# MaurizioFD/RecSys2019_DeepLearning_Evaluation

Measured on AMD Instinct MI355X. Metric: BPR-MF SGD samples/sec (k=128, batch 1000) + ItemKNN cosine build sec on ML-20M-shaped URM, higher is better.
Workload: dtype f32; 1 GPU; BPR-MF epoch (139 mini-batches x 1000 on-device samples), k=128, sgd, on synthetic ml20m URM 138493x26744 nnz=20001422; replicas (one independent model per GPU); batch_size=1000, n_factors=128, parallelism=replicas x1

## Files before the change

include/mi355rec.h:

```cpp
#ifndef MI355REC_H
#define MI355REC_H

#include <stdint.h>

#ifdef __cplusplus
extern "C" {
#endif

#define MI355REC_OK              0
#define MI355REC_E_INVALID      -1
#define MI355REC_E_HIP          -2
#define MI355REC_E_NO_DEVICE    -3
#define MI355REC_E_UNSUPPORTED  -4
#define MI355REC_E_NUMERIC      -5

const char *mi355rec_last_error(void);

int mi355rec_device_malloc(void **out, uint64_t bytes);
int mi355rec_device_free(void *p);
int mi355rec_device_memcpy(void *dst, const void *src, uint64_t bytes, int to_device);
int mi355rec_device_synchronize(void);
int mi355rec_device_trim(uint64_t *freed_bytes);
int mi355rec_device_count(int *count);
int mi355rec_set_device(int device);
// ... 108 lines not shown
    uint64_t random_seed;
    int32_t precision;
    int32_t reserved;
} mi355rec_mf_config;

typedef struct mi355rec_mf *mi355rec_mf_t;

int mi355rec_mf_create(mi355rec_mf_t *out, const mi355rec_mf_config *cfg, int32_t n_users, int32_t n_items,
                       const int32_t *indptr, const int32_t *indices, const float *data,
                       const void *U0, const void *V0);
int mi355rec_mf_run_epochs(mi355rec_mf_t h, int32_t n_epochs);
int mi355rec_mf_run_samples(mi355rec_mf_t h, const int32_t *u, const int32_t *i, const int32_t *j,
                            const float *rating, int64_t n);
int mi355rec_mf_shard_begin_epoch(mi355rec_mf_t h, int32_t rank, int32_t world, void **d_send, void **d_recv,
                                  uint64_t *bytes_per_rank, int32_t *n_batches);
int mi355rec_mf_shard_batch(mi355rec_mf_t h, int32_t batch);
int mi355rec_mf_shard_merge(mi355rec_mf_t h, int32_t batch);
int mi355rec_mf_shard_end_epoch(mi355rec_mf_t h);
int mi355rec_mf_get_factors(mi355rec_mf_t h, float *U, float *V, float *bu, float *bi, float *mu);
int mi355rec_mf_get_factors_f64(mi355rec_mf_t h, double *U, double *V, double *bu, double *bi, double *mu);
int mi355rec_mf_get_last_samples(mi355rec_mf_t h, int32_t *u, int32_t *i, int32_t *j, float *rating, int64_t cap, int64_t *n);
int mi355rec_mf_set_profiling(mi355rec_mf_t h, int32_t max_timed_launches);
int mi355rec_mf_get_phase_ticks(mi355rec_mf_t h, uint64_t *out, int64_t cap, int64_t *n);
int mi355rec_mf_get_stats(mi355rec_mf_t h, mi355rec_stats *stats);
void mi355rec_mf_destroy(mi355rec_mf_t h);

typedef struct mi355rec_mf_group *mi355rec_mf_group_t;
int mi355rec_mf_group_create(mi355rec_mf_group_t *out, const mi355rec_mf_t *members, int32_t n_members);
int mi355rec_mf_group_run_epochs(mi355rec_mf_group_t g, int32_t n_epochs);
int mi355rec_mf_group_set_profiling(mi355rec_mf_group_t g, int32_t max_timed_launches);
int mi355rec_mf_group_get_stats(mi355rec_mf_group_t g, mi355rec_stats *stats);
void mi355rec_mf_group_destroy(mi355rec_mf_group_t g);


typedef struct {
    int32_t symmetric;
    int32_t sgd_mode;
    double  learning_rate, li_reg, lj_reg;
    double  gamma, beta_1, beta_2;
    uint64_t random_seed;
    int32_t precision;
    int32_t train_with_sparse_weights;
    int32_t topK;
    int32_t reserved;
} mi355rec_slim_config;

// ... 201 lines not shown
```

recsys2019_deeplearning_evaluation_amd/_native.py:

```python
import ctypes as C
import os

import numpy as np

_HERE = os.path.dirname(os.path.abspath(__file__))
LIB_PATH = os.environ.get("MI355REC_LIB") or os.path.join(_HERE, "libmi355rec.so")

E_INVALID, E_HIP, E_NO_DEVICE, E_UNSUPPORTED, E_NUMERIC = -1, -2, -3, -4, -5

SIMILARITY_CODES = {"cosine": 0, "adjusted": 1, "asymmetric": 2, "pearson": 3, "jaccard": 4, "tanimoto": 4,
                    "dice": 5, "tversky": 6, "euclidean": 7}
EUCLIDEAN_MODE_CODES = {"lin": 0, "log": 1, "exp": 2}
FEATURE_WEIGHTING_CODES = {"none": 0, "BM25": 1, "TF-IDF": 2}
SGD_MODE_CODES = {"sgd": 0, "adagrad": 1, "rmsprop": 2, "adam": 3}
ALGORITHM_CODES = {"MF_BPR": 0, "FUNK_SVD": 1, "ASY_SVD": 2}
PRECISION_CODES = {"fp32": 0, "fp64": 1}


class NativeLibraryError(RuntimeError):
    """libmi355rec.so is missing, or the HIP runtime / device failed."""


class Stats(C.Structure):
    _fields_ = [("call_ms", C.c_double), ("kernel_ms", C.c_double), ("n_launches", C.c_int64), ("n_timed", C.c_int64),
# ... 63 lines not shown
    "mi355rec_sim_compute_dense_device": (C.c_int, [_vp, _i32, _i32, _vp, _i64]),
    "mi355rec_sim_compute_csr": (C.c_int, [_vp, C.c_int32, C.c_int32, _vp, _vp, _vp, _vp]),
    "mi355rec_sim_column_costs": (C.c_int, [_vp, _vp]),
    "mi355rec_sim_schedule_info": (C.c_int, [_vp, _vp, _vp, _vp]),
    "mi355rec_sim_accumulator_info": (C.c_int, [_vp, C.POINTER(_i32), C.POINTER(_f64)]),
    "mi355rec_sim_selection_info": (C.c_int, [_vp, C.POINTER(_i64), C.POINTER(_i64), C.POINTER(_i64)]),
    "mi355rec_lds_atomic_rate": (C.c_int, [C.POINTER(_f64)]),
    "mi355rec_sim_sync": (C.c_int, [_vp]),
    "mi355rec_sim_get_stats": (C.c_int, [_vp, C.POINTER(Stats)]),
    "mi355rec_sim_destroy": (None, [_vp]),
    "mi355rec_csr_stack_device": (C.c_int, [_i32, C.POINTER(CsrBlock), _i32, _vp, _vp, _vp]),
    "mi355rec_mf_create": (C.c_int, [C.POINTER(_vp), C.POINTER(MFConfig), _i32, _i32, _vp, _vp, _vp, _vp, _vp]),
    "mi355rec_mf_run_epochs": (C.c_int, [_vp, _i32]),
    "mi355rec_mf_run_samples": (C.c_int, [_vp, _vp, _vp, _vp, _vp, _i64]),
    "mi355rec_mf_shard_begin_epoch": (C.c_int, [_vp, _i32, _i32, C.POINTER(_vp), C.POINTER(_vp), C.POINTER(C.c_uint64), C.POINTER(_i32)]),
    "mi355rec_mf_shard_batch": (C.c_int, [_vp, _i32]),
    "mi355rec_mf_shard_merge": (C.c_int, [_vp, _i32]),
    "mi355rec_mf_shard_end_epoch": (C.c_int, [_vp]),
    "mi355rec_mf_get_factors": (C.c_int, [_vp, _vp, _vp, _vp, _vp, _vp]),
    "mi355rec_mf_get_factors_f64": (C.c_int, [_vp, _vp, _vp, _vp, _vp, _vp]),
    "mi355rec_mf_get_last_samples": (C.c_int, [_vp, _vp, _vp, _vp, _vp, _i64, C.POINTER(_i64)]),
    "mi355rec_mf_set_profiling": (C.c_int, [_vp, _i32]),
    "mi355rec_mf_get_phase_ticks": (C.c_int, [_vp, _vp, _i64, C.POINTER(_i64)]),
    "mi355rec_mf_get_stats": (C.c_int, [_vp, C.POINTER(Stats)]),
    "mi355rec_mf_destroy": (None, [_vp]),
    "mi355rec_mf_group_create": (C.c_int, [C.POINTER(_vp), C.POINTER(_vp), _i32]),
    "mi355rec_mf_group_run_epochs": (C.c_int, [_vp, _i32]),
    "mi355rec_mf_group_set_profiling": (C.c_int, [_vp, _i32]),
    "mi355rec_mf_group_get_stats": (C.c_int, [_vp, C.POINTER(Stats)]),
    "mi355rec_mf_group_destroy": (None, [_vp]),
    "mi355rec_slim_create": (C.c_int, [C.POINTER(_vp), C.POINTER(SlimConfig), _i32, _i32, _vp, _vp]),
    "mi355rec_slim_run_epochs": (C.c_int, [_vp, _i32]),
    "mi355rec_slim_run_samples": (C.c_int, [_vp, _vp, _vp, _vp, _i64]),
    "mi355rec_slim_get_last_samples": (C.c_int, [_vp, _vp, _vp, _vp, _i64, C.POINTER(_i64)]),
    "mi355rec_slim_get_S_topk": (C.c_int, [_vp, _i32, _vp, _vp]),
    "mi355rec_slim_get_W_csr": (C.c_int, [_vp, _i32, _vp, _vp, _vp, _vp, _vp, C.POINTER(C.c_int64)]),
    "mi355rec_slim_get_S_sparse": (C.c_int, [_vp, _vp, _vp]),
    "mi355rec_slim_get_S_dense": (C.c_int, [_vp, _vp]),
    "mi355rec_slim_get_stats": (C.c_int, [_vp, C.POINTER(Stats)]),
    "mi355rec_slim_schedule_info": (C.c_int, [_vp, C.POINTER(_i32), C.POINTER(_i32)]),
    "mi355rec_slim_destroy": (None, [_vp]),
    "mi355rec_ials_create": (C.c_int, [C.POINTER(_vp), _i32, _i32, _i32, _f64, _vp, _vp, _vp, _vp, _vp]),
    "mi355rec_ials_run_epochs": (C.c_int, [_vp, _i32]),
    "mi355rec_ials_user_half": (C.c_int, [_vp, _i32, _i32]),
    "mi355rec_ials_item_half": (C.c_int, [_vp, _i32, _i32]),
    "mi355rec_ials_device_factors": (C.c_int, [_vp, C.POINTER(_vp), C.POINTER(_vp)]),
# ... 391 lines not shown
```

recsys2019_deeplearning_evaluation_amd/csrc/mf.hip:

```cpp
#include "common.h"
#include "sampling.cuh"
#include "wave.cuh"

#include <rocprim/rocprim.hpp>

#include <memory>

#include "mf_core.cuh"
#include "mf_schedule.cuh"
#include "mf_batch.cuh"
#include "mf_asy.cuh"


using namespace mi355rec;

struct mi355rec_mf : Handle {
    mi355rec_mf_config cfg{};
    int n_users = 0, n_items = 0, k = 0;
    int n_u_rows = 0;
    bool f64 = false;
    size_t nnz = 0;
    DeviceBuffer<int> indptr, indices, su, si, sj;
    DeviceBuffer<float> data, sr, stage;
    DeviceBuffer<unsigned char> U[2], V[2], bu[2], bi[2], c1U, c2U, c1V, c2V, c1_bu, c2_bu, c1_bi, c2_bi;
    DeviceBuffer<unsigned char> mu_state, mu_acc, asy_mu, asy_c_mu;
    DeviceBuffer<unsigned char> par;
    DeviceBuffer<double> loss_slots;
    DeviceBuffer<MfState> state;
    DeviceBuffer<unsigned long long> keys, keys_sorted;
    DeviceBuffer<int> slots, slots_sorted, head, head_scan, task_at, batch_count;
    DeviceBuffer<unsigned char> spar, cub_tmp;
    DeviceBuffer<TaskHeader> tasks;
    DeviceBuffer<unsigned> touched;
    DeviceBuffer<int> sorted_slot, qtask, used;
    bool fast_schedule = false;
    DeviceBuffer<unsigned long long> ticks;
    DeviceBuffer<int4> recs, slot_recs;
    size_t cub_tmp_bytes = 0;
    size_t stream_capacity = 0;
    long long batch_capacity = 0;
    long long batches_done = 0;
    long long last_call_samples = 0;
    int max_timed = 0;
    DeviceBuffer<unsigned char> shard_send, shard_recv;
    int shard_rank = -1, shard_world = 0, shard_slots_per_rank = 0;
    long long shard_batches = 0;
    std::vector<hipGraphExec_t> epoch_graphs;
    size_t general_capacity = 0;
    bool graph_failed = false;
    std::vector<double> host_loss;

    void drop_graphs() {
        for (hipGraphExec_t g : epoch_graphs) (void)hipGraphExecDestroy(g);
        epoch_graphs.clear();
    }
    ~mi355rec_mf() { shutdown([&] { drop_graphs(); }); }
};

namespace {
// ... 157 lines not shown
}

FastSchedParams fast_sched_params(mi355rec_mf *h, long long n_samples) {
    FastSchedParams f;
    memset(&f, 0, sizeof(f));
    f.n_samples = n_samples;
    f.per = per_sample(h);
    f.n_users = h->n_users;
    f.n_entries = h->n_users + h->n_items;
    f.batch_size = h->cfg.batch_size;
    f.tasks_per_batch = f.per * h->cfg.batch_size;
    f.np = std::max(SCHED_THREADS, pow2_at_least(f.tasks_per_batch));
    f.slot_bits = bits_for((unsigned long long)f.np);
    f.entry_bits = std::min(32 - f.slot_bits, bits_for((unsigned long long)f.n_entries) + 1);
    f.mid_bytes = (int)sched_mid_bytes(f.np);
    f.words = FAST_MAX_BATCHES / 32;
    f.group = samples_in_flight(h);
    f.su = h->su.ptr; f.si = h->si.ptr; f.sj = h->sj.ptr; f.sr = h->sr.ptr;
    f.touched = h->touched.ptr; f.par = h->par.ptr;
    f.sorted_slot = h->sorted_slot.ptr; f.qtask = h->qtask.ptr; f.used = h->used.ptr;
    f.tasks = h->tasks.ptr; f.recs = h->recs.ptr; f.slot_recs = h->slot_recs.ptr;
    f.fuse = h->cfg.algorithm == MI355REC_MF_BPR && h->shard_rank < 0 && !getenv("MI355REC_MF_NO_FUSE");
    f.fill_all = 1;
    return f;
}

void enqueue_fast_schedule(mi355rec_mf *h, long long n_samples, long long n_batches, const FastSchedParams *given = nullptr,
                           hipStream_t on = nullptr) {
    hipStream_t s = on ? on : h->stream;
    const FastSchedParams f = given ? *given : fast_sched_params(h, n_samples);
    const size_t lds = sched_lds_bytes(f.np);
    static bool attr_set[64] = {};
    set_sched_sort_attribute(reinterpret_cast<const void *>(mf_sched_sort_kernel), attr_set);
    hipLaunchKernelGGL(mf_sched_sort_kernel, dim3((unsigned)n_batches), dim3(SCHED_THREADS), lds, s, f);
    hipLaunchKernelGGL(mf_sched_emit_kernel, dim3(div_up(f.batch_size, 256), (unsigned)n_batches), dim3(256), 0, s, f);
    hipLaunchKernelGGL(mf_sched_finish_kernel, dim3(div_up(f.n_entries, 256)), dim3(256), 0, s, f);
}

void enqueue_schedule(mi355rec_mf *h, long long n_samples, long long n_batches) {
    if (h->fast_schedule && fast_schedule_fits(h, n_batches)) {
        enqueue_fast_schedule(h, n_samples, n_batches);
        return;
    }
    hipStream_t s = h->stream;
    const int per = per_sample(h);
    const long long n = n_samples * per;
    SchedParams sp{};
// ... 17 lines not shown
    MI_REQUIRE(end_bit <= 64, "sample stream too long for the schedule keys");
    MI_HIP(hipMemsetAsync(h->batch_count.ptr, 0, sizeof(int) * (size_t)n_batches, s));
    MI_HIP(hipMemsetAsync(h->tasks.ptr, 0, sizeof(TaskHeader) * (size_t)n_batches * sp.tasks_per_batch, s));
    hipLaunchKernelGGL(mf_keys_kernel, dim3(div_up(n_samples, 256)), dim3(256), 0, s, sp);
    size_t bytes = h->cub_tmp_bytes;
    MI_HIP(rocprim::radix_sort_pairs(h->cub_tmp.ptr, bytes, h->keys.ptr, h->keys_sorted.ptr, h->slots.ptr,
                                              h->slots_sorted.ptr, (int)n, 0, end_bit, s));
    MI_HIP(hipMemsetAsync(sp.slot_flag, 0, sizeof(int) * (size_t)n, s));
    hipLaunchKernelGGL(mf_heads_kernel, dim3(div_up(n, 256)), dim3(256), 0, s, sp);
    bytes = h->cub_tmp_bytes;
    MI_HIP(rocprim::inclusive_scan(h->cub_tmp.ptr, bytes, h->head.ptr, h->head_scan.ptr, (size_t)n, rocprim::plus<int>(), s));
    bytes = h->cub_tmp_bytes;
    MI_HIP(rocprim::exclusive_scan(h->cub_tmp.ptr, bytes, sp.slot_flag, reinterpret_cast<int *>(h->keys.ptr) + n, 0, (size_t)n, rocprim::plus<int>(), s));
    hipLaunchKernelGGL(mf_tasks_kernel, dim3(div_up(n, 256)), dim3(256), 0, s, sp);
    hipLaunchKernelGGL(mf_recs_kernel, dim3(div_up(n, 256)), dim3(256), 0, s, sp);
}

long long schedule_span(const mi355rec_mf *h, long long n_batches) {
    if (h->shard_rank < 0 && n_batches > FAST_MAX_BATCHES && fast_schedule_fits(h, 1) && !getenv("MI355REC_MF_WHOLE_STREAM_SCHEDULE"))
        return FAST_MAX_BATCHES;
    return n_batches;
}

template <class T>
void enqueue_stream(mi355rec_mf *h, const MfParams<T> &p, long long n_samples, long long n_batches, bool timed, long long first = 0,
                    long long last = -1) {
    const bool bpr = h->cfg.algorithm == MI355REC_MF_BPR;
    const long long span = schedule_span(h, n_batches), B = h->cfg.batch_size;
    if (last < 0) last = n_batches;
    for (long long b = first; b < last; ++b) {
        const long long part = b / span * span, local = b - part, part_batches = std::min(span, n_batches - part);
        if (local == 0) {
            if (span == n_batches) {
                enqueue_schedule(h, n_samples, n_batches);
            } else {
                FastSchedParams f = fast_sched_params(h, std::min(n_samples - part * B, part_batches * B));
                f.su += part * B; f.si += part * B; f.sj += part * B; f.sr += part * B;
                enqueue_fast_schedule(h, f.n_samples, part_batches, &f);
            }
        }
        if (bpr) launch_batch<MI355REC_MF_BPR, T>(h, p, (int)local, timed);
        else launch_batch<MI355REC_MF_FUNK_SVD, T>(h, p, (int)local, timed);
        if (local + 1 == part_batches) hipLaunchKernelGGL(mf_stream_end_kernel<T>, dim3(1), dim3(64), 0, h->stream, p, part_batches);
    }
}

constexpr int ASY_CHUNK = 1 << 16;

template <class T>
void enqueue_asy_steps(mi355rec_mf *h, const MfParams<T> &p, long long n_steps, bool timed) {
    for (long long first = 0; first < n_steps; first += ASY_CHUNK) {
        const int count = (int)std::min<long long>(ASY_CHUNK, n_steps - first);
        hipEvent_t e0 = nullptr, e1 = nullptr;
        if (timed) h->dispatch_timers.next(e0, e1, h->max_timed);
        auto go = [&](auto kernel) {
            if (e0) hipExtLaunchKernelGGL(kernel, dim3(1), dim3(1024), 0, h->stream, e0, e1, 0, p, first, count);
            else hipLaunchKernelGGL(kernel, dim3(1), dim3(1024), 0, h->stream, p, first, count);
        };
        if (h->k <= 64) go(mf_asy_kernel<T, 1>);
        else if (h->k <= 128) go(mf_asy_kernel<T, 2>);
        else go(mf_asy_kernel<T, 4>);
    }
}

template <class T>
void enqueue_epoch(mi355rec_mf *h, const MfParams<T> &p, bool timed, long long first = 0, long long last = -1) {
    if (first == 0) launch_sampler(h, p);
    if (h->cfg.algorithm == MI355REC_MF_ASY_SVD) {
        enqueue_asy_steps(h, p, p.samples_per_epoch, timed);
        return;
    }
    enqueue_stream(h, p, p.samples_per_epoch, batches_per_epoch(h), timed, first, last);
}

constexpr long long GRAPH_SEGMENT = 4096, MAX_GRAPH_BATCHES = 64 * GRAPH_SEGMENT;
template <class T>
void ensure_epoch_graph(mi355rec_mf *h, const MfParams<T> &p) {
    if (!h->epoch_graphs.empty() || h->graph_failed) return;
    const long long nb = h->cfg.algorithm == MI355REC_MF_ASY_SVD ? 1 : batches_per_epoch(h);
    for (long long first = 0; first < nb; first += GRAPH_SEGMENT) {
        hipGraph_t g = nullptr;
        hipGraphExec_t exec = nullptr;
        hipError_t e = hipStreamBeginCapture(h->stream, hipStreamCaptureModeThreadLocal);
        if (e == hipSuccess) {
            try {
                enqueue_epoch(h, p, false, first, std::min(nb, first + GRAPH_SEGMENT));
            } catch (...) {
                (void)hipStreamEndCapture(h->stream, &g);
                if (g) (void)hipGraphDestroy(g);
                (void)hipGetLastError();
                h->drop_graphs();
                h->graph_failed = true;
                return;
            }
            e = hipStreamEndCapture(h->stream, &g);
// ... 221 lines not shown
        MI_REQUIRE(cfg->sgd_mode >= MI355REC_SGD && cfg->sgd_mode <= MI355REC_ADAM, "Value for 'sgd_mode' not recognized (%d)",
                   cfg->sgd_mode);
        MI_REQUIRE(cfg->n_factors >= 1, "n_factors must be >= 1");
        if (cfg->n_factors > 512) fail(MI355REC_E_UNSUPPORTED, "n_factors = %d exceeds 512", cfg->n_factors);
        MI_REQUIRE(cfg->batch_size >= 1, "batch_size must be >= 1");
        MI_REQUIRE(cfg->precision == MI355REC_F32 || cfg->precision == MI355REC_F64, "precision must be MI355REC_F32 or MI355REC_F64");
        ensure_device();
        std::unique_ptr<mi355rec_mf> h(new mi355rec_mf());
        h->cfg = *cfg;
        h->n_users = n_users;
        h->n_items = n_items;
        h->k = cfg->n_factors;
        h->n_u_rows = asy ? n_items : n_users;
        h->f64 = cfg->precision == MI355REC_F64;
        h->nnz = (size_t)indptr[n_users];
        MI_REQUIRE(h->nnz > 0, "URM has no interactions");
        h->open(1);
        hipStream_t s = h->stream;
        h->indptr.upload(indptr, (size_t)n_users + 1, s);
        h->indices.upload(indices, h->nnz, s);
        h->data.upload(data, h->nnz, s);
        if (h->f64) create_typed<double>(h.get(), U0, V0); else create_typed<float>(h.get(), U0, V0);
        h->par.alloc_zero((size_t)n_users + n_items, s);
        if (getenv("MI355REC_MF_TICKS")) h->ticks.alloc_zero((size_t)per_sample(h.get()) * cfg->batch_size * 8, s);
        h->loss_slots.alloc_zero((size_t)per_sample(h.get()) * cfg->batch_size * 4, s);
        h->state.alloc_zero(1, s);
        {
            MfState init{};
            init.beta_1_power = cfg->beta_1;
            init.beta_2_power = cfg->beta_2;
            MI_HIP(hipMemcpyAsync(h->state.ptr, &init, sizeof(MfState), hipMemcpyHostToDevice, s));
        }
        MI_HIP(hipStreamSynchronize(s));
        *out = h.release();
    });
}

extern "C" int mi355rec_mf_run_epochs(mi355rec_mf_t h, int32_t n_epochs) {
    return guarded([&] {
        MI_REQUIRE(h, "NULL handle");
        MI_REQUIRE(n_epochs >= 0, "n_epochs must be >= 0");
        ensure_device();
        ReleaseScope scope(h->stream);
        if (h->f64) run_epochs_typed<double>(h, n_epochs); else run_epochs_typed<float>(h, n_epochs);
    });
}

// ... 503 lines not shown

extern "C" int mi355rec_mf_set_profiling(mi355rec_mf_t h, int32_t max_timed_launches) {
    return guarded([&] {
        MI_REQUIRE(h, "NULL handle");
        MI_REQUIRE(max_timed_launches >= 0 && max_timed_launches <= 65536, "max_timed_launches out of range");
        ensure_device();
        h->max_timed = max_timed_launches;
        h->dispatch_timers.reserve(max_timed_launches);
    });
}

extern "C" int mi355rec_mf_get_phase_ticks(mi355rec_mf_t h, uint64_t *out, int64_t cap, int64_t *n) {
    return guarded([&] {
        MI_REQUIRE(h && n, "NULL argument");
        ensure_device();
        *n = (int64_t)h->ticks.count;
        if (out && cap > 0) {
            MI_HIP(hipStreamSynchronize(h->stream));
            MI_HIP(hipMemcpy(out, h->ticks.ptr, sizeof(uint64_t) * std::min<size_t>((size_t)cap, h->ticks.count), hipMemcpyDeviceToHost));
        }
    });
}

extern "C" int mi355rec_mf_get_stats(mi355rec_mf_t h, mi355rec_stats *stats) { return handle_get_stats(h, stats); }

extern "C" void mi355rec_mf_destroy(mi355rec_mf_t h) { handle_destroy(h); }
```

recsys2019_deeplearning_evaluation_amd/csrc/mf_core.cuh:

```cuda
#pragma once

namespace mi355rec {
namespace {


struct MfState {
    long long batch_base;
    long long epoch;
    double beta_1_power, beta_2_power;
    double asy_loss;
};

struct TaskHeader {
    int entry;
    int meta;
    int start;
    int pad;
    int4 rec0;
};
constexpr int LEN_MASK = 0x0fffffff;
typedef int int8v __attribute__((ext_vector_type(8)));
constexpr int ROLE_U = 0, ROLE_I = 1;

template <class T> struct MuState { T mu, c1, c2, pad; };
// ... 73 lines not shown

template <class T> __device__ __forceinline__ T grad_term(T scale, T x, T reg, T w) {
#pragma clang fp contract(off)
    const T a = scale * x;
    const T b = reg * w;
    return a - b;
}
__device__ __forceinline__ float fused_add(float a, float b, float c) { return __builtin_fmaf(a, b, c); }
__device__ __forceinline__ double fused_add(double a, double b, double c) { return __builtin_fma(a, b, c); }
template <class T> __device__ __forceinline__ T diff_of(T a, T b) {
#pragma clang fp contract(off)
    return a - b;
}
template <class T> __device__ __forceinline__ T mean_of(T sum, T inv_batch) {
#pragma clang fp contract(off)
    return sum * inv_batch;
}
template <class T> __device__ __forceinline__ T moved(T w, T lr, T step) {
#pragma clang fp contract(off)
    const T a = lr * step;
    return w + a;
}

template <int ALGO, class T>
__device__ __forceinline__ void mf_sample_body(const MfParams<T> &p) {
    const long long t = blockIdx.x * (long long)blockDim.x + threadIdx.x;
    const long long epoch = p.state->epoch;
    if (t < p.samples_per_epoch) {
        const unsigned long long sid = (unsigned long long)(epoch * p.samples_per_epoch + t);
        unsigned d = 0;
        int u, start = 0, n_seen = 0;
        do {
            u = bounded(draw32(p.seed, sid, d++), p.n_users);
            start = p.indptr[u];
            n_seen = p.indptr[u + 1] - start;
        } while (n_seen == 0 || n_seen == p.n_items);
        const int *row = p.indices + start;
        p.su[t] = u;
        if (ALGO == MI355REC_MF_BPR) {
            p.si[t] = row[bounded(draw32(p.seed, sid, d++), n_seen)];
            int j;
            do { j = bounded(draw32(p.seed, sid, d++), p.n_items); } while (!profile_lacks(row, n_seen, j));
            p.sj[t] = j;
        } else {
            bool positive = true;
            if (p.sample_negatives) positive = (float)draw32(p.seed, sid, d++) * 2.3283064365386963e-10f <= p.quota;
            if (positive) {
                const int at = bounded(draw32(p.seed, sid, d++), n_seen);
                p.si[t] = row[at];
                p.sr[t] = p.data[start + at];
            } else {
                int i;
                do { i = bounded(draw32(p.seed, sid, d++), p.n_items); } while (!profile_lacks(row, n_seen, i));
                p.si[t] = i;
                p.sr[t] = 0.f;
            }
        }
    }
}
template <int ALGO, class T>
__global__ __launch_bounds__(256) void mf_sample_kernel(const MfParams<T> p) { mf_sample_body<ALGO, T>(p); }
__global__ void mf_epoch_advance_kernel(MfState *state) {
    if (threadIdx.x == 0 && blockIdx.x == 0) state->epoch += 1;
}

}
}
```

recsys2019_deeplearning_evaluation_amd/csrc/mf_schedule.cuh:

```cuda
#pragma once

namespace mi355rec {
namespace {

struct SchedParams {
    long long n_samples;
    int per;
    int n_users, batch_size, batch_bits, tasks_per_batch;
    const int *su, *si, *sj;
    const float *sr;
    unsigned long long *keys;
    int *slots;
    const unsigned long long *keys_sorted;
    const int *slots_sorted;
    int *head;
    const int *head_scan;
    int *task_at;
    unsigned char *spar;
    unsigned char *par;
    int *batch_count;
    int *slot_flag;
    const int *slot_rank;
    TaskHeader *tasks;
    int4 *recs;
// ... 62 lines not shown
    if (q >= n) return;
    const int slot = s.slots_sorted[q];
    const int sample = slot / s.per, role = slot - sample * s.per;
    const long long base = (long long)sample * s.per;
    int4 rec;
    rec.x = s.su[sample];
    rec.y = s.si[sample];
    rec.z = s.per == 3 ? s.sj[sample] : __float_as_int(s.sr[sample]);
    rec.w = role | (s.spar[base] << 2) | (s.spar[base + 1] << 3) | (s.per == 3 ? s.spar[base + 2] << 4 : 0);
    s.recs[q] = rec;
    if (s.head[q]) {
        s.tasks[s.task_at[q]].rec0 = rec;
        const int entry = (int)(s.keys_sorted[q] >> s.batch_bits);
        long long end = q + 1;
        while (end < n && !s.head[end]) ++end;
        if (end == n || (int)(s.keys_sorted[end] >> s.batch_bits) != entry) s.par[entry] = s.spar[slot] ^ 1;
    }
}

constexpr int META_WIDE = 1 << 30;
constexpr int SCHED_THREADS = 1024;
constexpr int SLOT_ABSORBED = 0x3fffffff;
constexpr int FAST_MAX_BATCHES = 256, FAST_MAX_SLOTS = 8192;

struct FastSchedParams {
    long long n_samples;
    int per, n_users, n_entries, batch_size, tasks_per_batch, slot_bits, np, words, group;
    int fill_all;
    int mid_bytes;
    int entry_bits;
    int fuse;
    const int *su, *si, *sj;
    const float *sr;
    unsigned *touched;
    unsigned char *par;
    int *sorted_slot;
    int *qtask;
    int *used;
    TaskHeader *tasks;
    int4 *recs;
    int4 *slot_recs;
};

template <int IPT> struct SchedSort {
    using type = rocprim::block_radix_sort<unsigned, SCHED_THREADS, IPT>;
    static __device__ __forceinline__ void run(unsigned *K, void *storage, int begin_bit, int end_bit) {
        unsigned keys[IPT];
#pragma unroll
        for (int i = 0; i < IPT; ++i) keys[i] = K[threadIdx.x * IPT + i];
        type().sort(keys, *reinterpret_cast<typename type::storage_type *>(storage), (unsigned)begin_bit, (unsigned)end_bit);
        __syncthreads();
#pragma unroll
        for (int i = 0; i < IPT; ++i) K[threadIdx.x * IPT + i] = keys[i];
    }
};
constexpr size_t sched_sort_storage_bytes(int np) {
    return np <= SCHED_THREADS ? sizeof(SchedSort<1>::type::storage_type)
           : (np <= 2 * SCHED_THREADS ? sizeof(SchedSort<2>::type::storage_type)
              : (np <= 4 * SCHED_THREADS ? sizeof(SchedSort<4>::type::storage_type) : sizeof(SchedSort<8>::type::storage_type)));
}

__device__ __forceinline__ void mf_sched_sort_body(const FastSchedParams &s, const int b) {
    extern __shared__ __attribute__((aligned(16))) unsigned sched_lds[];
    unsigned *K = sched_lds;
    int *hpos = reinterpret_cast<int *>(sched_lds + s.np);
    int *tpos = hpos + s.np + 1;
    typedef rocprim::block_scan<int, SCHED_THREADS> Scan;
    __shared__ typename Scan::storage_type scan_tmp;
    const int tid = threadIdx.x, np = s.np, sb = s.slot_bits;
    const long long first = (long long)b * s.batch_size;
    const int n_in = (int)min((long long)s.batch_size, s.n_samples - first);
    const int m = n_in * s.per;
    for (int q = tid; q < np; q += SCHED_THREADS) {
        unsigned key = 0xFFFFFFFFu;
        if (q < m) {
            const int smp = q / s.per, role = q - smp * s.per;
            const long long t = first + smp;
            const int entry = role == 0 ? s.su[t] : s.n_users + (role == 1 ? s.si[t] : s.sj[t]);
            key = ((unsigned)entry << sb) | (unsigned)q;
        }
        K[q] = key;
    }
    __syncthreads();
    switch (np / SCHED_THREADS) {
        case 1: SchedSort<1>::run(K, hpos, sb, sb + s.entry_bits); break;
        case 2: SchedSort<2>::run(K, hpos, sb, sb + s.entry_bits); break;
        case 4: SchedSort<4>::run(K, hpos, sb, sb + s.entry_bits); break;
        default: SchedSort<8>::run(K, hpos, sb, sb + s.entry_bits); break;
    }
    __syncthreads();
    const int C = np / SCHED_THREADS;
    int cnt = 0;
    for (int c = 0; c < C; ++c) {
        const int q = tid * C + c;
        cnt += q < m && (q == 0 || (K[q] >> sb) != (K[q - 1] >> sb));
    }
    int off = 0, total = 0;
    Scan().exclusive_scan(cnt, off, 0, total, scan_tmp);
    for (int c = 0; c < C; ++c) {
        const int q = tid * C + c;
        if (q < m && (q == 0 || (K[q] >> sb) != (K[q - 1] >> sb))) hpos[off++] = q;
    }
    if (tid == 0) hpos[total] = m;
    __syncthreads();
    unsigned char *single = reinterpret_cast<unsigned char *>(sched_lds) + sizeof(unsigned) * (size_t)np + s.mid_bytes;
    const unsigned qmask = (1u << sb) - 1u;
    if (s.fuse) {
        for (int q = tid; q < np; q += SCHED_THREADS) single[q] = 0;
        __syncthreads();
        for (int t = tid; t < total; t += SCHED_THREADS)
            if (hpos[t + 1] - hpos[t] == 1) single[K[hpos[t]] & qmask] = 1;
        __syncthreads();
    }
    auto absorbed = [&](int t) -> bool {
        if (!s.fuse || hpos[t + 1] - hpos[t] != 1) return false;
        const int inc = (int)(K[hpos[t]] & qmask), smp = inc / s.per;
        return inc != smp * s.per && single[smp * s.per];
    };
    auto lone_user = [&](int q) -> bool {
        if (q >= m) return false;
        const unsigned e = K[q] >> sb;
        return e < (unsigned)s.n_users && (q == 0 || (K[q - 1] >> sb) != e) && (q + 1 == m || (K[q + 1] >> sb) != e);
    };
    auto paired = [&](int q) -> bool {
        if (!s.fuse || s.group < 2) return false;
        const int q0 = q - q % s.group;
        for (int e = 0; e < s.group; ++e)
            if (!lone_user(q0 + e)) return false;
        return true;
    };
    const int CT = (total + SCHED_THREADS - 1) / SCHED_THREADS;
    const int t_lo = min(tid * CT, total), t_hi = min(t_lo + CT, total);
    int wcnt = 0, acnt = 0;
    const int wide_min = 2 * s.group;
    for (int t = t_lo; t < t_hi; ++t) {
        const int start = hpos[t], len = hpos[t + 1] - start;
        wcnt += len > wide_min;
        acnt += absorbed(t) || (len == 1 && start % s.group != 0 && paired(start));
    }
    int woff = 0, n_wide = 0, aoff = 0, n_abs = 0;
    Scan().exclusive_scan(wcnt, woff, 0, n_wide, scan_tmp);
    __syncthreads();
    Scan().exclusive_scan(acnt, aoff, 0, n_abs, scan_tmp);
    TaskHeader *out = s.tasks + (size_t)b * s.tasks_per_batch;
    for (int t = t_lo; t < t_hi; ++t) {
        const int start = hpos[t], len = hpos[t + 1] - start;
        const bool wide = len > wide_min;
        const int entry = (int)(K[start] >> sb);
        atomicOr(&s.touched[(size_t)entry * s.words + (b >> 5)], 1u << (b & 31));
        const bool pair = len == 1 && paired(start);
        if (absorbed(t) || (pair && start % s.group != 0)) {
            ++aoff;
            tpos[t] = SLOT_ABSORBED;
            continue;
        }
        const int slot = wide ? 4 * woff : 4 * n_wide + (t - woff - aoff);
        woff += wide;
        tpos[t] = slot | (wide ? META_WIDE : 0);
        for (int part = 0; part < (wide ? 4 : 1); ++part) {
            *reinterpret_cast<int4 *>(out + slot + part) =
                make_int4(entry, (pair ? s.group : len) | (wide ? META_WIDE | (part << 28) : 0), b * s.tasks_per_batch + start, pair ? 1 : 0);
            out[slot + part].rec0 = make_int4(0, 0, 0, 0);
        }
    }
    const int used = 4 * n_wide + (total - n_wide - n_abs);
    if (tid == 0) s.used[b] = used;
    const int fill_end = s.fill_all ? s.tasks_per_batch : min(s.tasks_per_batch, (used + 3) & ~3);
    for (int slot = used + tid; slot < fill_end; slot += SCHED_THREADS)
        *reinterpret_cast<int4 *>(out + slot) = make_int4(0, 0, 0, 0);
    __syncthreads();
    for (int q = tid; q < m; q += SCHED_THREADS) {
        int lo = 0, hi = total;
        while (hi - lo > 1) {
            const int mid = (lo + hi) >> 1;
            if (hpos[mid] <= q) lo = mid; else hi = mid;
        }
        const int inc = (int)(K[q] & qmask);
        int also = 0;
        if (s.fuse && hpos[lo + 1] - hpos[lo] == 1) {
            const int smp = inc / s.per;
            if (inc == smp * s.per) also = (single[inc + 1] ? 1 : 0) | (s.per == 3 && single[inc + 2] ? 2 : 0);
        }
        s.sorted_slot[(size_t)b * s.tasks_per_batch + inc] = q | (also << 16);
        s.qtask[(size_t)b * s.tasks_per_batch + q] = tpos[lo];
    }
}
__global__ __launch_bounds__(SCHED_THREADS) void mf_sched_sort_kernel(const FastSchedParams s) { mf_sched_sort_body(s, blockIdx.x); }

__device__ __forceinline__ int version_parity(const FastSchedParams &s, int entry, int b) {
    const unsigned *w = s.touched + (size_t)entry * s.words;
    int cnt = 0;
    for (int k = 0; k < (b >> 5); ++k) cnt += __popc(w[k]);
    cnt += __popc(w[b >> 5] & ((1u << (b & 31)) - 1u));
    return (s.par[entry] + cnt) & 1;
}

__device__ __forceinline__ void mf_sched_emit_body(const FastSchedParams &s) {
    const int b = blockIdx.y, smp = blockIdx.x * 256 + threadIdx.x;
    const long long first = (long long)b * s.batch_size;
    const int n_in = (int)min((long long)s.batch_size, s.n_samples - first);
    if (smp >= n_in) return;
    const size_t base = (size_t)b * s.tasks_per_batch;
    const long long t = first + smp;
    const int u = s.su[t], i = s.si[t], j = s.per == 3 ? s.sj[t] : 0;
    const int third = s.per == 3 ? j : __float_as_int(s.sr[t]);
    int where[3];
#pragma unroll
    for (int role = 0; role < 3; ++role) where[role] = role < s.per ? s.sorted_slot[base + (size_t)smp * s.per + role] : 0;
    const int pu = version_parity(s, u, b), pi = version_parity(s, s.n_users + i, b);
    const int pj = s.per == 3 ? version_parity(s, s.n_users + j, b) : 0;
    const int par_bits = (pu << 2) | (pi << 3) | (pj << 4);
#pragma unroll
    for (int role = 0; role < 3; ++role) {
        if (role >= s.per) break;
        const int q = where[role] & 0xffff, also = where[role] >> 16;
        const size_t at = base + q;
        const int4 rec = make_int4(u, i, third, role | par_bits | (also << 5));
        s.recs[at] = rec;
        const int tp = s.qtask[at];
        if (tp == SLOT_ABSORBED) {
            const int q0 = q - q % s.group;
            if (s.fuse && q0 != q) {
                const int tp0 = s.qtask[base + q0];
                if (tp0 != SLOT_ABSORBED && !(tp0 & META_WIDE)) {
                    const TaskHeader *lead = s.tasks + base + tp0;
                    if (lead->pad == 1 && lead->start == (int)(base + q0)) s.slot_recs[(base + tp0) * 3 + (q - q0 - 1)] = rec;
                }
            }
            continue;
        }
        TaskHeader *hd = s.tasks + base + (tp & (META_WIDE - 1));
        const int off = (int)(at - (size_t)hd->start);
        const int own = role == 0 ? pu : (role == 1 ? pi : pj);
        int part = -1;
        if (tp & META_WIDE) {
            if (off % s.group == 0 && off / s.group < 4) part = off / s.group;
        } else if (off == 0) {
            part = 0;
        }
        if (part >= 0) {
            hd[part].rec0 = rec;
            hd[part].meta |= own << 31;
        }
    }
}

__global__ __launch_bounds__(256) void mf_sched_emit_kernel(const FastSchedParams s) { mf_sched_emit_body(s); }

__device__ __forceinline__ void mf_sched_finish_body(const FastSchedParams &s) {
    const int x = blockIdx.x * 256 + threadIdx.x;
    if (x >= s.n_entries) return;
    unsigned *w = s.touched + (size_t)x * s.words;
    int cnt = 0;
    for (int k = 0; k < s.words; ++k) {
        const unsigned v = w[k];
        if (v) { cnt += __popc(v); w[k] = 0; }
    }
    if (cnt & 1) s.par[x] ^= 1;
}
__global__ __launch_bounds__(256) void mf_sched_finish_kernel(const FastSchedParams s) { mf_sched_finish_body(s); }

template <class T>
__device__ __forceinline__ void ring_to_stream_start(const MfParams<T> &p, const long long n_batches, const int slot) {
    if (n_batches <= 0) return;
    const int src = (int)((n_batches - 1) % 3);
    if (src != 2) {
        if (slot == 0) p.mu_state[2] = p.mu_state[src];
        p.mu_acc[2 * MU_SLOTS + slot] = p.mu_acc[src * MU_SLOTS + slot];
    }
    p.mu_acc[slot] = (T)0;
}

template <class T>
// ... 17 lines not shown
```

Measured before the change: 225.9 million samples/s.

## Fuse BPR sample drawing into schedule sort kernel and streamline emit lookups

When the whole epoch fits the fast schedule, the separate sampler kernel launch is skipped and samples are drawn inside the per-batch schedule sort kernel, which writes the sort keys directly. The finish kernel advances the epoch counter instead. The emit kernel now loads touched bitmaps as uint4 with an unrolled popcount, and reads the task offset and pair flag packed into qtask rather than dereferencing task headers. Optional schedule timestamp probes are added behind an env var. The risks are heavier work per sort block, since drawing is serialised into 1024-thread blocks per batch, and the hardcoded 8-word bitmap stride and packed qtask bit fields.

```diff
diff --git a/include/mi355rec.h b/include/mi355rec.h
--- a/include/mi355rec.h
+++ b/include/mi355rec.h
@@ -154,6 +154,7 @@
 int mi355rec_mf_get_last_samples(mi355rec_mf_t h, int32_t *u, int32_t *i, int32_t *j, float *rating, int64_t cap, int64_t *n);
 int mi355rec_mf_set_profiling(mi355rec_mf_t h, int32_t max_timed_launches);
 int mi355rec_mf_get_phase_ticks(mi355rec_mf_t h, uint64_t *out, int64_t cap, int64_t *n);
+int mi355rec_mf_get_schedule_ticks(mi355rec_mf_t h, uint64_t *out, int64_t cap, int64_t *n);
 int mi355rec_mf_get_stats(mi355rec_mf_t h, mi355rec_stats *stats);
 void mi355rec_mf_destroy(mi355rec_mf_t h);
 
diff --git a/recsys2019_deeplearning_evaluation_amd/_native.py b/recsys2019_deeplearning_evaluation_amd/_native.py
--- a/recsys2019_deeplearning_evaluation_amd/_native.py
+++ b/recsys2019_deeplearning_evaluation_amd/_native.py
@@ -109,6 +109,7 @@
     "mi355rec_mf_get_last_samples": (C.c_int, [_vp, _vp, _vp, _vp, _vp, _i64, C.POINTER(_i64)]),
     "mi355rec_mf_set_profiling": (C.c_int, [_vp, _i32]),
     "mi355rec_mf_get_phase_ticks": (C.c_int, [_vp, _vp, _i64, C.POINTER(_i64)]),
+    "mi355rec_mf_get_schedule_ticks": (C.c_int, [_vp, _vp, _i64, C.POINTER(_i64)]),
     "mi355rec_mf_get_stats": (C.c_int, [_vp, C.POINTER(Stats)]),
     "mi355rec_mf_destroy": (None, [_vp]),
     "mi355rec_mf_group_create": (C.c_int, [C.POINTER(_vp), C.POINTER(_vp), _i32]),
diff --git a/recsys2019_deeplearning_evaluation_amd/csrc/mf.hip b/recsys2019_deeplearning_evaluation_amd/csrc/mf.hip
--- a/recsys2019_deeplearning_evaluation_amd/csrc/mf.hip
+++ b/recsys2019_deeplearning_evaluation_amd/csrc/mf.hip
@@ -34,7 +34,7 @@
     DeviceBuffer<unsigned> touched;
     DeviceBuffer<int> sorted_slot, qtask, used;
     bool fast_schedule = false;
-    DeviceBuffer<unsigned long long> ticks;
+    DeviceBuffer<unsigned long long> ticks, sched_ticks;
     DeviceBuffer<int4> recs, slot_recs;
     size_t cub_tmp_bytes = 0;
     size_t stream_capacity = 0;
@@ -238,7 +238,25 @@
     f.tasks = h->tasks.ptr; f.recs = h->recs.ptr; f.slot_recs = h->slot_recs.ptr;
     f.fuse = h->cfg.algorithm == MI355REC_MF_BPR && h->shard_rank < 0 && !getenv("MI355REC_MF_NO_FUSE");
     f.fill_all = 1;
+    f.ticks = h->sched_ticks.ptr;
     return f;
+}
+
+bool schedule_draws(const mi355rec_mf *h);
+
+template <class T>
+void set_draw(FastSchedParams &f, const MfParams<T> &p) {
+    f.draw = 1;
+    f.advance_epoch = 1;
+    f.bpr = f.per == 3;
+    f.sample_negatives = p.sample_negatives;
+    f.n_items = p.n_items;
+    f.quota = p.quota;
+    f.seed = p.seed;
+    f.samples_per_epoch = p.samples_per_epoch;
+    f.first_sample = 0;
+    f.state = p.state;
+    f.indptr = p.indptr; f.indices = p.indices; f.data = p.data;
 }
 
 void enqueue_fast_schedule(mi355rec_mf *h, long long n_samples, long long n_batches, const FastSchedParams *given = nullptr,
@@ -302,16 +320,26 @@
     return n_batches;
 }
 
+bool schedule_draws(const mi355rec_mf *h) {
+    const long long nb = batches_per_epoch(h);
+    return h->cfg.algorithm != MI355REC_MF_ASY_SVD && h->shard_rank < 0 && h->fast_schedule && fast_schedule_fits(h, nb) &&
+           schedule_span(h, nb) == nb;
+}
+
 template <class T>
 void enqueue_stream(mi355rec_mf *h, const MfParams<T> &p, long long n_samples, long long n_batches, bool timed, long long first = 0,
-                    long long last = -1) {
+                    long long last = -1, bool draw = false) {
     const bool bpr = h->cfg.algorithm == MI355REC_MF_BPR;
     const long long span = schedule_span(h, n_batches), B = h->cfg.batch_size;
     if (last < 0) last = n_batches;
     for (long long b = first; b < last; ++b) {
         const long long part = b / span * span, local = b - part, part_batches = std::min(span, n_batches - part);
         if (local == 0) {
-            if (span == n_batches) {
+            if (draw) {
+                FastSchedParams f = fast_sched_params(h, n_samples);
+                set_draw(f, p);
+                enqueue_fast_schedule(h, n_samples, n_batches, &f);
+            } else if (span == n_batches) {
                 enqueue_schedule(h, n_samples, n_batches);
             } else {
                 FastSchedParams f = fast_sched_params(h, std::min(n_samples - part * B, part_batches * B));
@@ -345,12 +373,13 @@
 
 template <class T>
 void enqueue_epoch(mi355rec_mf *h, const MfParams<T> &p, bool timed, long long first = 0, long long last = -1) {
-    if (first == 0) launch_sampler(h, p);
+    const bool draw = schedule_draws(h);
+    if (first == 0 && !draw) launch_sampler(h, p);
     if (h->cfg.algorithm == MI355REC_MF_ASY_SVD) {
         enqueue_asy_steps(h, p, p.samples_per_epoch, timed);
         return;
     }
-    enqueue_stream(h, p, p.samples_per_epoch, batches_per_epoch(h), timed, first, last);
+    enqueue_stream(h, p, p.samples_per_epoch, batches_per_epoch(h), timed, first, last, draw);
 }
 
 constexpr long long GRAPH_SEGMENT = 4096, MAX_GRAPH_BATCHES = 64 * GRAPH_SEGMENT;
@@ -618,7 +647,10 @@
         h->data.upload(data, h->nnz, s);
         if (h->f64) create_typed<double>(h.get(), U0, V0); else create_typed<float>(h.get(), U0, V0);
         h->par.alloc_zero((size_t)n_users + n_items, s);
-        if (getenv("MI355REC_MF_TICKS")) h->ticks.alloc_zero((size_t)per_sample(h.get()) * cfg->batch_size * 8, s);
+        if (getenv("MI355REC_MF_TICKS")) {
+            h->ticks.alloc_zero((size_t)per_sample(h.get()) * cfg->batch_size * 8, s);
+            h->sched_ticks.alloc_zero((size_t)FAST_MAX_BATCHES * SCHED_STAMPS, s);
+        }
         h->loss_slots.alloc_zero((size_t)per_sample(h.get()) * cfg->batch_size * 4, s);
         h->state.alloc_zero(1, s);
         {
@@ -1168,6 +1200,18 @@
     });
 }
 
+extern "C" int mi355rec_mf_get_schedule_ticks(mi355rec_mf_t h, uint64_t *out, int64_t cap, int64_t *n) {
+    return guarded([&] {
+        MI_REQUIRE(h && n, "NULL argument");
+        ensure_device();
+        *n = (int64_t)h->sched_ticks.count;
+        if (out && cap > 0) {
+            MI_HIP(hipStreamSynchronize(h->stream));
+            MI_HIP(hipMemcpy(out, h->sched_ticks.ptr, sizeof(uint64_t) * std::min<size_t>((size_t)cap, h->sched_ticks.count), hipMemcpyDeviceToHost));
+        }
+    });
+}
+
 extern "C" int mi355rec_mf_get_stats(mi355rec_mf_t h, mi355rec_stats *stats) { return handle_get_stats(h, stats); }
 
 extern "C" void mi355rec_mf_destroy(mi355rec_mf_t h) { handle_destroy(h); }
diff --git a/recsys2019_deeplearning_evaluation_amd/csrc/mf_core.cuh b/recsys2019_deeplearning_evaluation_amd/csrc/mf_core.cuh
--- a/recsys2019_deeplearning_evaluation_amd/csrc/mf_core.cuh
+++ b/recsys2019_deeplearning_evaluation_amd/csrc/mf_core.cuh
@@ -119,40 +119,49 @@
     return w + a;
 }
 
+__device__ __forceinline__ void mf_draw_sample(const bool bpr, const unsigned long long seed, const unsigned long long sid, const int n_users,
+                                               const int n_items, const int *indptr, const int *indices, const float *data,
+                                               const int sample_negatives, const float quota, int &u, int &i, int &third) {
+    unsigned d = 0;
+    int start = 0, n_seen = 0;
+    do {
+        u = bounded(draw32(seed, sid, d++), n_users);
+        start = indptr[u];
+        n_seen = indptr[u + 1] - start;
+    } while (n_seen == 0 || n_seen == n_items);
+    const int *row = indices + start;
+    if (bpr) {
+        i = row[bounded(draw32(seed, sid, d++), n_seen)];
+        int j;
+        do { j = bounded(draw32(seed, sid, d++), n_items); } while (!profile_lacks(row, n_seen, j));
+        third = j;
+    } else {
+        bool positive = true;
+        if (sample_negatives) positive = (float)draw32(seed, sid, d++) * 2.3283064365386963e-10f <= quota;
+        if (positive) {
+            const int at = bounded(draw32(seed, sid, d++), n_seen);
+            i = row[at];
+            third = __float_as_int(data[start + at]);
+        } else {
+            do { i = bounded(draw32(seed, sid, d++), n_items); } while (!profile_lacks(row, n_seen, i));
+            third = __float_as_int(0.f);
+        }
+    }
+}
+
 template <int ALGO, class T>
 __device__ __forceinline__ void mf_sample_body(const MfParams<T> &p) {
     const long long t = blockIdx.x * (long long)blockDim.x + threadIdx.x;
     const long long epoch = p.state->epoch;
     if (t < p.samples_per_epoch) {
         const unsigned long long sid = (unsigned long long)(epoch * p.samples_per_epoch + t);
-        unsigned d = 0;
-        int u, start = 0, n_seen = 0;
-        do {
-            u = bounded(draw32(p.seed, sid, d++), p.n_users);
-            start = p.indptr[u];
-            n_seen = p.indptr[u + 1] - start;
-        } while (n_seen == 0 || n_seen == p.n_items);
-        const int *row = p.indices + start;
+        int u, i, third;
+        mf_draw_sample(ALGO == MI355REC_MF_BPR, p.seed, sid, p.n_users, p.n_items, p.indptr, p.indices, p.data, p.sample_negatives, p.quota,
+                       u, i, third);
         p.su[t] = u;
-        if (ALGO == MI355REC_MF_BPR) {
-            p.si[t] = row[bounded(draw32(p.seed, sid, d++), n_seen)];
-            int j;
-            do { j = bounded(draw32(p.seed, sid, d++), p.n_items); } while (!profile_lacks(row, n_seen, j));
-            p.sj[t] = j;
-        } else {
-            bool positive = true;
-            if (p.sample_negatives) positive = (float)draw32(p.seed, sid, d++) * 2.3283064365386963e-10f <= p.quota;
-            if (positive) {
-                const int at = bounded(draw32(p.seed, sid, d++), n_seen);
-                p.si[t] = row[at];
-                p.sr[t] = p.data[start + at];
-            } else {
-                int i;
-                do { i = bounded(draw32(p.seed, sid, d++), p.n_items); } while (!profile_lacks(row, n_seen, i));
-                p.si[t] = i;
-                p.sr[t] = 0.f;
-            }
-        }
+        p.si[t] = i;
+        if (ALGO == MI355REC_MF_BPR) p.sj[t] = third;
+        else p.sr[t] = __int_as_float(third);
     }
 }
 template <int ALGO, class T>
diff --git a/recsys2019_deeplearning_evaluation_amd/csrc/mf_schedule.cuh b/recsys2019_deeplearning_evaluation_amd/csrc/mf_schedule.cuh
--- a/recsys2019_deeplearning_evaluation_amd/csrc/mf_schedule.cuh
+++ b/recsys2019_deeplearning_evaluation_amd/csrc/mf_schedule.cuh
@@ -108,6 +108,8 @@
 constexpr int SCHED_THREADS = 1024;
 constexpr int SLOT_ABSORBED = 0x3fffffff;
 constexpr int FAST_MAX_BATCHES = 256, FAST_MAX_SLOTS = 8192;
+constexpr int QTASK_SLOT_MASK = FAST_MAX_SLOTS - 1, QTASK_OFF_SHIFT = 13, QTASK_OFF_MAX = 31, QTASK_PAIR = 1 << 29;
+constexpr int SCHED_STAMPS = 8;
 
 struct FastSchedParams {
     long long n_samples;
@@ -116,8 +118,16 @@
     int mid_bytes;
     int entry_bits;
     int fuse;
-    const int *su, *si, *sj;
-    const float *sr;
+    int *su, *si, *sj;
+    float *sr;
+    int draw, advance_epoch, bpr, sample_negatives, n_items;
+    float quota;
+    unsigned long long seed;
+    long long samples_per_epoch, first_sample;
+    MfState *state;
+    const int *indptr, *indices;
+    const float *data;
+    unsigned long long *ticks;
     unsigned *touched;
     unsigned char *par;
     int *sorted_slot;
@@ -157,17 +167,40 @@
     const long long first = (long long)b * s.batch_size;
     const int n_in = (int)min((long long)s.batch_size, s.n_samples - first);
     const int m = n_in * s.per;
-    for (int q = tid; q < np; q += SCHED_THREADS) {
-        unsigned key = 0xFFFFFFFFu;
-        if (q < m) {
-            const int smp = q / s.per, role = q - smp * s.per;
+    auto mark = [&](int phase) {
+        if (s.ticks && tid == 0) s.ticks[(size_t)b * SCHED_STAMPS + phase] = stamp();
+    };
+    mark(0);
+    if (s.draw) {
+        const unsigned long long sid0 = (unsigned long long)(s.state->epoch * s.samples_per_epoch + s.first_sample + first);
+        for (int smp = tid; smp < n_in; smp += SCHED_THREADS) {
+            int u, i, third;
+            mf_draw_sample(s.bpr != 0, s.seed, sid0 + (unsigned long long)smp, s.n_users, s.n_items, s.indptr, s.indices, s.data,
+                           s.sample_negatives, s.quota, u, i, third);
             const long long t = first + smp;
-            const int entry = role == 0 ? s.su[t] : s.n_users + (role == 1 ? s.si[t] : s.sj[t]);
-            key = ((unsigned)entry << sb) | (unsigned)q;
-        }
-        K[q] = key;
+            s.su[t] = u;
+            s.si[t] = i;
+            if (s.bpr) s.sj[t] = third; else s.sr[t] = __int_as_float(third);
+            const int q = smp * s.per;
+            K[q] = ((unsigned)u << sb) | (unsigned)q;
+            K[q + 1] = ((unsigned)(s.n_users + i) << sb) | (unsigned)(q + 1);
+            if (s.per == 3) K[q + 2] = ((unsigned)(s.n_users + third) << sb) | (unsigned)(q + 2);
+        }
+        for (int q = m + tid; q < np; q += SCHED_THREADS) K[q] = 0xFFFFFFFFu;
+    } else {
+        for (int q = tid; q < np; q += SCHED_THREADS) {
+            unsigned key = 0xFFFFFFFFu;
+            if (q < m) {
+                const int smp = q / s.per, role = q - smp * s.per;
+                const long long t = first + smp;
+                const int entry = role == 0 ? s.su[t] : s.n_users + (role == 1 ? s.si[t] : s.sj[t]);
+                key = ((unsigned)entry << sb) | (unsigned)q;
+            }
+            K[q] = key;
+        }
     }
     __syncthreads();
+    mark(1);
     switch (np / SCHED_THREADS) {
         case 1: SchedSort<1>::run(K, hpos, sb, sb + s.entry_bits); break;
         case 2: SchedSort<2>::run(K, hpos, sb, sb + s.entry_bits); break;
@@ -175,6 +208,7 @@
         default: SchedSort<8>::run(K, hpos, sb, sb + s.entry_bits); break;
     }
     __syncthreads();
+    mark(2);
     const int C = np / SCHED_THREADS;
     int cnt = 0;
     for (int c = 0; c < C; ++c) {
@@ -189,6 +223,7 @@
     }
     if (tid == 0) hpos[total] = m;
     __syncthreads();
+    mark(3);
     unsigned char *single = reinterpret_cast<unsigned char *>(sched_lds) + sizeof(unsigned) * (size_t)np + s.mid_bytes;
     const unsigned qmask = (1u << sb) - 1u;
     if (s.fuse) {
@@ -215,6 +250,7 @@
             if (!lone_user(q0 + e)) return false;
         return true;
     };
+    mark(4);
     const int CT = (total + SCHED_THREADS - 1) / SCHED_THREADS;
     const int t_lo = min(tid * CT, total), t_hi = min(t_lo + CT, total);
     int wcnt = 0, acnt = 0;
@@ -228,6 +264,7 @@
     Scan().exclusive_scan(wcnt, woff, 0, n_wide, scan_tmp);
     __syncthreads();
     Scan().exclusive_scan(acnt, aoff, 0, n_abs, scan_tmp);
+    mark(5);
     TaskHeader *out = s.tasks + (size_t)b * s.tasks_per_batch;
     for (int t = t_lo; t < t_hi; ++t) {
         const int start = hpos[t], len = hpos[t + 1] - start;
@@ -242,7 +279,7 @@
         }
         const int slot = wide ? 4 * woff : 4 * n_wide + (t - woff - aoff);
         woff += wide;
-        tpos[t] = slot | (wide ? META_WIDE : 0);
+        tpos[t] = slot | (wide ? META_WIDE : 0) | (pair ? QTASK_PAIR : 0);
         for (int part = 0; part < (wide ? 4 : 1); ++part) {
             *reinterpret_cast<int4 *>(out + slot + part) =
                 make_int4(entry, (pair ? s.group : len) | (wide ? META_WIDE | (part << 28) : 0), b * s.tasks_per_batch + start, pair ? 1 : 0);
@@ -255,6 +292,7 @@
     for (int slot = used + tid; slot < fill_end; slot += SCHED_THREADS)
         *reinterpret_cast<int4 *>(out + slot) = make_int4(0, 0, 0, 0);
     __syncthreads();
+    mark(6);
     for (int q = tid; q < m; q += SCHED_THREADS) {
         int lo = 0, hi = total;
         while (hi - lo > 1) {
@@ -268,17 +306,30 @@
             if (inc == smp * s.per) also = (single[inc + 1] ? 1 : 0) | (s.per == 3 && single[inc + 2] ? 2 : 0);
         }
         s.sorted_slot[(size_t)b * s.tasks_per_batch + inc] = q | (also << 16);
-        s.qtask[(size_t)b * s.tasks_per_batch + q] = tpos[lo];
-    }
+        const int tp = tpos[lo];
+        s.qtask[(size_t)b * s.tasks_per_batch + q] = tp == SLOT_ABSORBED ? tp : tp | (min(q - hpos[lo], QTASK_OFF_MAX) << QTASK_OFF_SHIFT);
+    }
+    mark(7);
 }
 __global__ __launch_bounds__(SCHED_THREADS) void mf_sched_sort_kernel(const FastSchedParams s) { mf_sched_sort_body(s, blockIdx.x); }
 
-__device__ __forceinline__ int version_parity(const FastSchedParams &s, int entry, int b) {
-    const unsigned *w = s.touched + (size_t)entry * s.words;
+struct RowBits { uint4 lo, hi; };
+__device__ __forceinline__ RowBits row_bits(const FastSchedParams &s, int entry) {
+    const uint4 *w = reinterpret_cast<const uint4 *>(s.touched + (size_t)entry * (FAST_MAX_BATCHES / 32));
+    RowBits r;
+    r.lo = w[0];
+    r.hi = w[1];
+    return r;
+}
+__device__ __forceinline__ int version_parity(const RowBits &r, int par, int b) {
+    const unsigned w[8] = {r.lo.x, r.lo.y, r.lo.z, r.lo.w, r.hi.x, r.hi.y, r.hi.z, r.hi.w};
     int cnt = 0;
-    for (int k = 0; k < (b >> 5); ++k) cnt += __popc(w[k]);
-    cnt += __popc(w[b >> 5] & ((1u << (b & 31)) - 1u));
-    return (s.par[entry] + cnt) & 1;
+#pragma unroll
+    for (int k = 0; k < 8; ++k) {
+        const unsigned mask = k < (b >> 5) ? 0xFFFFFFFFu : (k == (b >> 5) ? (1u << (b & 31)) - 1u : 0u);
+        cnt += __popc(w[k] & mask);
+    }
+    return (par + cnt) & 1;
 }
 
 __device__ __forceinline__ void mf_sched_emit_body(const FastSchedParams &s) {
@@ -288,13 +339,26 @@
     if (smp >= n_in) return;
     const size_t base = (size_t)b * s.tasks_per_batch;
     const long long t = first + smp;
-    const int u = s.su[t], i = s.si[t], j = s.per == 3 ? s.sj[t] : 0;
-    const int third = s.per == 3 ? j : __float_as_int(s.sr[t]);
+    const bool three = s.per == 3;
+    const int u = s.su[t], i = s.si[t], j = s.sj[t];
+    const int rating = __float_as_int(s.sr[t]);
     int where[3];
 #pragma unroll
-    for (int role = 0; role < 3; ++role) where[role] = role < s.per ? s.sorted_slot[base + (size_t)smp * s.per + role] : 0;
-    const int pu = version_parity(s, u, b), pi = version_parity(s, s.n_users + i, b);
-    const int pj = s.per == 3 ? version_parity(s, s.n_users + j, b) : 0;
+    for (int role = 0; role < 3; ++role) where[role] = s.sorted_slot[base + (size_t)smp * s.per + (role < s.per ? role : 0)];
+    const int third = three ? j : rating;
+    const int ej = s.n_users + (three ? j : i);
+    const RowBits bu = row_bits(s, u), bi = row_bits(s, s.n_users + i), bj = row_bits(s, ej);
+    const int su0 = s.par[u], si0 = s.par[s.n_users + i], sj0 = s.par[ej];
+    const int gmask = s.group - 1, gshift = s.group >> 1;
+    int tps[3], tps0[3];
+#pragma unroll
+    for (int role = 0; role < 3; ++role) {
+        const int q = where[role] & 0xffff;
+        tps[role] = s.qtask[base + q];
+        tps0[role] = s.qtask[base + (q & ~gmask)];
+    }
+    const int pu = version_parity(bu, su0, b), pi = version_parity(bi, si0, b);
+    const int pj = three ? version_parity(bj, sj0, b) : 0;
     const int par_bits = (pu << 2) | (pi << 3) | (pj << 4);
 #pragma unroll
     for (int role = 0; role < 3; ++role) {
@@ -303,30 +367,25 @@
         const size_t at = base + q;
         const int4 rec = make_int4(u, i, third, role | par_bits | (also << 5));
         s.recs[at] = rec;
-        const int tp = s.qtask[at];
+        const int tp = tps[role];
         if (tp == SLOT_ABSORBED) {
-            const int q0 = q - q % s.group;
-            if (s.fuse && q0 != q) {
-                const int tp0 = s.qtask[base + q0];
-                if (tp0 != SLOT_ABSORBED && !(tp0 & META_WIDE)) {
-                    const TaskHeader *lead = s.tasks + base + tp0;
-                    if (lead->pad == 1 && lead->start == (int)(base + q0)) s.slot_recs[(base + tp0) * 3 + (q - q0 - 1)] = rec;
-                }
-            }
+            const int q0 = q & ~gmask, tp0 = tps0[role];
+            if (s.fuse && q0 != q && tp0 != SLOT_ABSORBED && (tp0 & QTASK_PAIR))
+                s.slot_recs[(base + (tp0 & QTASK_SLOT_MASK)) * 3 + (q - q0 - 1)] = rec;
             continue;
         }
-        TaskHeader *hd = s.tasks + base + (tp & (META_WIDE - 1));
-        const int off = (int)(at - (size_t)hd->start);
+        TaskHeader *hd = s.tasks + base + (tp & QTASK_SLOT_MASK);
+        const int off = (tp >> QTASK_OFF_SHIFT) & QTASK_OFF_MAX;
         const int own = role == 0 ? pu : (role == 1 ? pi : pj);
         int part = -1;
         if (tp & META_WIDE) {
-            if (off % s.group == 0 && off / s.group < 4) part = off / s.group;
+            if ((off & gmask) == 0 && (off >> gshift) < 4) part = off >> gshift;
         } else if (off == 0) {
             part = 0;
         }
         if (part >= 0) {
             hd[part].rec0 = rec;
-            hd[part].meta |= own << 31;
+            if (own) hd[part].meta |= (int)(1u << 31);
         }
     }
 }
@@ -335,6 +394,7 @@
 
 __device__ __forceinline__ void mf_sched_finish_body(const FastSchedParams &s) {
     const int x = blockIdx.x * 256 + threadIdx.x;
+    if (s.advance_epoch && x == 0) s.state->epoch += 1;
     if (x >= s.n_entries) return;
     unsigned *w = s.touched + (size_t)x * s.words;
     int cnt = 0;
```

Measured after the change: 229.8 million samples/s (median of 6 runs). 1.7% higher.
